# uci-cbcl/esm-efficient

Measured on AMD Instinct MI355X. Metric: residues/sec ESM2-650M fwd, 50k packed tokens; % bf16 MFMA peak; 1/2/4/8 GPU, higher is better.
Workload: dtype bf16

## Files before the change

### esm-efficient_amd/csrc/attn.hip

```cpp
#include "common.h"
#include "launch.h"
#include "gemm.h"

#include <atomic>
#include <type_traits>

namespace esme {

static constexpr int QT = 128;
static constexpr int KT = 64;
static constexpr int kAttnDma0 = 3, kAttnDma1 = 11;

struct AttnArgs {
    const u16* q; const u16* k; const u16* v; int64_t ld;
    u16* o; int64_t ldo;
    const int32_t* cu;
    int H;
    float scale_log2;
    int nqt;
    int nhb;
    float thr;
    int spec;
    const int32_t* order;
};

template <int D>
__device__ __forceinline__ int kswz(int row) {
    constexpr int CPR = D / 8;
    constexpr int RPB = 16 / CPR;
    return (row / RPB) & (CPR - 1);
}

template <int D, int QB, bool F16 = false>
__global__ __launch_bounds__(256, 2) void attn_varlen_kernel(const AttnArgs a) {
    constexpr int DS = D / 16;
    constexpr int DB = (D + 31) / 32;
    constexpr int CPR = D / 8;
    constexpr int KCH = KT * CPR;
    constexpr int KI = (KCH + 255) / 256;
    constexpr int DQ = D / 4;
    constexpr int DQ_HI_BITS = (D == 16 ? 0 : D == 32 ? 1 : D == 64 ? 2 : 3);
    constexpr int VI = (16 * DQ + 255) / 256;
    constexpr int K_BYTES = KT * D * 2;
    constexpr int BUF = K_BYTES + D * 128;
    const float THR = a.thr;

    __shared__ __attribute__((aligned(16))) char smem[2 * BUF];

    const int tid = threadIdx.x, lane = tid & 63, wave = tid >> 6;
    const int l31 = lane & 31, hi = lane >> 5;
    const int b = a.order ? a.order[blockIdx.z] : (int)blockIdx.z, h = blockIdx.y;
    const int s0 = a.cu[b], S = a.cu[b + 1] - s0;
    const int q0 = blockIdx.x * (QT * QB);
    if (q0 >= S) return;

    const unsigned int ld = (unsigned int)a.ld;
    const u16* qb = a.q + (int64_t)s0 * a.ld + h * D;
    const u16* kb = a.k + (int64_t)s0 * a.ld + h * D;
    const u16* vb = a.v + (int64_t)s0 * a.ld + h * D;

    int qrow[QB];
    bool blk_active[QB];
    bf16x8 qf[QB][DS];
#pragma unroll
    for (int b = 0; b < QB; ++b) {
        const int r0 = q0 + (wave * QB + b) * 32;
        qrow[b] = r0 + l31;
        blk_active[b] = r0 < S;
        const unsigned int qc = qrow[b] < S ? qrow[b] : S - 1;
#pragma unroll
        for (int ds = 0; ds < DS; ++ds)
            qf[b][ds] = *reinterpret_cast<const bf16x8*>(qb + (qc * ld + ds * 16 + hi * 8));
    }
    const bool wave_active = blk_active[0];

    unsigned int koff[KI];
    int krow[KI];
#pragma unroll
    for (int i = 0; i < KI; ++i) {
        const int c = i * 256 + tid;
        krow[i] = c / CPR;
        koff[i] = (unsigned int)(c % CPR) * 8u;
    }
    int v_dq[VI], v_kq[VI];
#pragma unroll
    for (int i = 0; i < VI; ++i) {
        const int rest = (lane >> 4) | (wave << 2) | (i << 4);
        v_dq[i] = (lane & 3) | ((rest & ((1 << DQ_HI_BITS) - 1)) << 2);
        v_kq[i] = ((lane >> 2) & 3) | ((rest >> DQ_HI_BITS) << 2);
    }
    u32x4 kreg[KI];
    u32x2 vreg[VI][4];
    auto load_tile = [&](int kv0) {
        const bool full = kv0 + KT <= S;
#pragma unroll
        for (int i = 0; i < KI; ++i) {
            if (KCH >= 256 * KI || krow[i] < KT) {
                unsigned int row = kv0 + krow[i];
                if (!full) row = row < (unsigned int)S ? row : S - 1;
                kreg[i] = *reinterpret_cast<const u32x4*>(kb + (row * ld + koff[i]));
            }
        }
#pragma unroll
        for (int i = 0; i < VI; ++i) {
            if (v_kq[i] < 16) {
#pragma unroll
                for (int kk = 0; kk < 4; ++kk) {
                    unsigned int row = kv0 + v_kq[i] * 4 + kk;
                    if (!full) row = row < (unsigned int)S ? row : S - 1;
                    vreg[i][kk] = *reinterpret_cast<const u32x2*>(vb + (row * ld + v_dq[i] * 4));
                }
            }
        }
    };
    auto store_tile = [&](char* Ks, char* Vt) {
#pragma unroll
        for (int i = 0; i < KI; ++i) {
            if (KCH >= 256 * KI || krow[i] < KT) {
                const int row = krow[i], ch = (int)(koff[i] >> 3);
                ESME_LDS_CHECK(Ks + row * (D * 2) + ((ch ^ kswz<D>(row)) << 4), 16, smem, 2 * BUF);
                *reinterpret_cast<u32x4*>(Ks + row * (D * 2) + ((ch ^ kswz<D>(row)) << 4)) = kreg[i];
            }
        }
#pragma unroll
        for (int i = 0; i < VI; ++i) {
            if (v_kq[i] < 16) {
                const int dq = v_dq[i], kq = v_kq[i];
#pragma unroll
                for (int dd = 0; dd < 4; ++dd) {
                    const int w = dd >> 1;
                    unsigned int e0, e1;
                    if (dd & 1) {
                        e0 = __builtin_amdgcn_perm(vreg[i][1][w], vreg[i][0][w], 0x07060302u);
                        e1 = __builtin_amdgcn_perm(vreg[i][3][w], vreg[i][2][w], 0x07060302u);
                    } else {
                        e0 = __builtin_amdgcn_perm(vreg[i][1][w], vreg[i][0][w], 0x05040100u);
                        e1 = __builtin_amdgcn_perm(vreg[i][3][w], vreg[i][2][w], 0x05040100u);
                    }
                    const int drow = dq * 4 + dd;
                    const int ch = kq >> 1;
                    u32x2 out = {e0, e1};
                    ESME_LDS_CHECK(Vt + drow * 128 + ((ch ^ ((drow >> 1) & 7)) << 4) + (kq & 1) * 8, 8, smem, 2 * BUF);
                    *reinterpret_cast<u32x2*>(Vt + drow * 128 + ((ch ^ ((drow >> 1) & 7)) << 4) + (kq & 1) * 8) = out;
                }
            }
        }
    };

    const int krow_perm = (l31 & 3) | (((l31 >> 3) & 1) << 2) | (((l31 >> 2) & 1) << 3) | (l31 & 16);

    f32x16 oacc[QB][DB];
    float mc[QB], l_run[QB];
#pragma unroll
    for (int b = 0; b < QB; ++b) {
        mc[b] = -1e30f; l_run[b] = 0.f;
#pragma unroll
        for (int i = 0; i < DB; ++i)
#pragma unroll
            for (int r = 0; r < 16; ++r) oacc[b][i][r] = 0.f;
    }
    const float c = a.scale_log2;

    const int ntiles = (S + KT - 1) / KT;
    load_tile(0);
// ... 242 lines not shown
                        const int drow = dq * 4 + dd;
                        const int ch = kq >> 1;
                        u32x2 out = {e0, e1};
                        ESME_LDS_CHECK(Vt + drow * 128 + ((ch ^ ((drow >> 1) & 7)) << 4) + (kq & 1) * 8, 8, smem, 2 * BUF);
                        *reinterpret_cast<u32x2*>(Vt + drow * 128 + ((ch ^ ((drow >> 1) & 7)) << 4) + (kq & 1) * 8) = out;
                    }
                }
            }
        }
    };

    const int krow_perm = (l31 & 3) | (((l31 >> 3) & 1) << 2) | (((l31 >> 2) & 1) << 3) | (l31 & 16);

    f32x16 oacc[DB];
    float mc = -1e30f, l_run = 0.f;
#pragma unroll
    for (int i = 0; i < DB; ++i)
#pragma unroll
        for (int r = 0; r < 16; ++r) oacc[i][r] = 0.f;
    const float c = a.scale_log2;

    const int ntiles = (S + KT - 1) / KT;
    load_tile(0);
    store_tile(smem);
    if (ntiles > 1) load_tile(KT);
    __syncthreads();
    for (int t = 0; t < ntiles; ++t) {
        const int kv0 = t * KT;
        const char* buf = smem + (t & 1) * BUF;
        if (wave_active) {
            f32x16 sacc[2];
#pragma unroll
            for (int kbk = 0; kbk < 2; ++kbk) {
#pragma unroll
                for (int r = 0; r < 16; ++r) sacc[kbk][r] = 0.f;
                const int row = kbk * 32 + krow_perm;
                const char* rp = buf + row * (D * 2);
                const int sw = kswz<D>(row);
#pragma unroll
                for (int ds = 0; ds < DS; ++ds) {
                    const bf16x8 kh = *reinterpret_cast<const bf16x8*>(rp + (((ds * 2 + hi) ^ sw) << 4));
                    ESME_LDS_CHECK(rp + K_BYTES + (((ds * 2 + hi) ^ sw) << 4), 16, smem, 2 * BUF);
                    const bf16x8 kl = *reinterpret_cast<const bf16x8*>(rp + K_BYTES + (((ds * 2 + hi) ^ sw) << 4));
                    sacc[kbk] = mfma_32x32x16<F16>(kl, qf[0][ds], sacc[kbk]);
                    sacc[kbk] = mfma_32x32x16<F16>(kh, qf[1][ds], sacc[kbk]);
                    sacc[kbk] = mfma_32x32x16<F16>(kh, qf[0][ds], sacc[kbk]);
                }
            }
            if (kv0 + KT > S) {
#pragma unroll
                for (int kbk = 0; kbk < 2; ++kbk)
#pragma unroll
                    for (int r = 0; r < 16; ++r)
                        if (kv0 + kbk * 32 + 16 * (r >> 3) + 8 * hi + (r & 7) >= S) sacc[kbk][r] = -1e30f;
            }
            float tmax = sacc[0][0];
#pragma unroll
            for (int r = 1; r < 16; ++r) tmax = fmaxf(tmax, sacc[0][r]);
#pragma unroll
            for (int r = 0; r < 16; ++r) tmax = fmaxf(tmax, sacc[1][r]);
            tmax = fmaxf(tmax, __shfl_xor(tmax, 32, 64));
            const float tmc = tmax * c;
            if (__any(tmc > mc)) {
                const float mn = fmaxf(mc, tmc);
                const float alpha = __builtin_amdgcn_exp2f(mc - mn);
                mc = mn;
                l_run *= alpha;
#pragma unroll
                for (int i = 0; i < DB; ++i)
#pragma unroll
                    for (int r = 0; r < 16; ++r) oacc[i][r] *= alpha;
            }
            bf16x8 pf[NPT][2][2];
            float psum = 0.f;
#pragma unroll
            for (int kbk = 0; kbk < 2; ++kbk)
#pragma unroll
                for (int s = 0; s < 2; ++s) {
                    float p[8], ph[8];
#pragma unroll
                    for (int j = 0; j < 8; ++j) {
                        p[j] = __builtin_amdgcn_exp2f(fmaf(sacc[kbk][8 * s + j], c, -mc));
                        psum += p[j];
                    }
                    const u32x4 pk = pack8t<F16>(p);
                    pf[0][kbk][s] = __builtin_bit_cast(bf16x8, pk);
                    if constexpr (!QKP) {
                        unpack8t<F16>(pk, ph);
#pragma unroll
                        for (int j = 0; j < 8; ++j) p[j] -= ph[j];
                        pf[NPT - 1][kbk][s] = __builtin_bit_cast(bf16x8, pack8t<F16>(p));
                    }
                }
            l_run += psum;

            const char* Vt = buf + 2 * K_BYTES;
#pragma unroll
            for (int i = 0; i < DB; ++i) {
                int drow = i * 32 + l31;
                if (D < 32) drow &= (D - 1);
                const char* rp = Vt + drow * 128;
                const int sw = (drow >> 1) & 7;
#pragma unroll
                for (int kbk = 0; kbk < 2; ++kbk)
#pragma unroll
                    for (int s = 0; s < 2; ++s) {
                        const bf16x8 vh = *reinterpret_cast<const bf16x8*>(rp + (((kbk * 4 + s * 2 + hi) ^ sw) << 4));
                        if constexpr (!QKP) {
                            ESME_LDS_CHECK(rp + V_BYTES + (((kbk * 4 + s * 2 + hi) ^ sw) << 4), 16, smem, 2 * BUF);
                            const bf16x8 vl = *reinterpret_cast<const bf16x8*>(rp + V_BYTES + (((kbk * 4 + s * 2 + hi) ^ sw) << 4));
                            oacc[i] = mfma_32x32x16<F16>(vl, pf[0][kbk][s], oacc[i]);
                            oacc[i] = mfma_32x32x16<F16>(vh, pf[NPT - 1][kbk][s], oacc[i]);
                        }
                        oacc[i] = mfma_32x32x16<F16>(vh, pf[0][kbk][s], oacc[i]);
                    }
            }
        }
        if (t + 1 < ntiles) {
            store_tile(smem + ((t + 1) & 1) * BUF);
            if (t + 2 < ntiles) load_tile(kv0 + 2 * KT);
        }
        __syncthreads();
    }

    if (!wave_active) return;
    const float l_tot = l_run + __shfl_xor(l_run, 32, 64);
    const float inv = 1.0f / l_tot;
    if (qrow < S) {
        u16* op = a.o + (int64_t)(s0 + qrow) * a.ldo + h * D;
#pragma unroll
        for (int i = 0; i < DB; ++i)
#pragma unroll
            for (int g = 0; g < 4; ++g) {
                const int d = i * 32 + 8 * g + 4 * hi;
                if (d < D) {
                    float o4[4];
#pragma unroll
                    for (int e = 0; e < 4; ++e) o4[e] = oacc[i][4 * g + e] * inv;
                    const u32x2 pk = {pack16<F16>(o4[0], o4[1]), pack16<F16>(o4[2], o4[3])};
                    *reinterpret_cast<u32x2*>(op + d) = pk;
                    if constexpr (!QKP) {
                        const u32x2 pl = {pack16<F16>(o4[0] - lo16<F16>(pk[0]), o4[1] - hi16<F16>(pk[0])), pack16<F16>(o4[2] - lo16<F16>(pk[1]), o4[3] - hi16<F16>(pk[1]))};
                        *reinterpret_cast<u32x2*>(op + sa.lo_out + d) = pl;
                    }
                }
            }
    }
}


template <int NW, bool QP = false, int D = 64, bool F16 = false>
__global__ __launch_bounds__(NW * 64, 2) void attn_pp64_kernel(const AttnArgs a) {
    constexpr float S0 = (QP && F16) ? -4.0f : 0.0f;
    constexpr int DS = D / 16, DB = D / 32, NT = NW * 64;
    constexpr int ROWB = D * 2;
    constexpr int K_BYTES = KT * D * 2;
    constexpr int SLOT = K_BYTES + D * 128;
    constexpr int ROWS = NW * 64;
    constexpr int NPV = 4 * DB, NQK = 2 * DS, NM = NPV + NQK;
    constexpr int PPS = 16 / NM;
    static_assert(D == 64 || D == 32, "head dims 64 and 32");
    static_assert(NW == 4 || (NW == 8 && D == 64), "4 waves (8: head dim 64 only)");
    extern __shared__ __attribute__((aligned(16))) char smem[];

    const int tid = threadIdx.x, lane = tid & 63;
    const int wave = __builtin_amdgcn_readfirstlane(tid >> 6);
    const int l31 = lane & 31, hi = lane >> 5;
    const unsigned int xcd = blockIdx.x & 7u, bi = blockIdx.x >> 3;
    const int qt = (int)(bi % (unsigned int)a.nqt);
    const unsigned int hb = (bi / (unsigned int)a.nqt) * 8u + xcd;
    if (hb >= (unsigned int)a.nhb) return;
    const int h = (int)(hb % (unsigned int)a.H), bi_seq = (int)(hb / (unsigned int)a.H);
    const int b = a.order ? a.order[bi_seq] : bi_seq;
    const int s0 = a.cu[b], S = a.cu[b + 1] - s0;
    const int q0 = qt * ROWS;
    if (q0 >= S) return;

    const unsigned int ld = (unsigned int)a.ld;
    const u16* qb = a.q + (int64_t)s0 * a.ld + h * D;
    const unsigned int kv_bytes = ((unsigned int)(S - 1) * ld + D) * 2u;
    auto make_rsrc = [&](const u16* p) -> u32x4 {
        const uint64_t v = (uint64_t)(uintptr_t)p;
        return u32x4{(unsigned int)__builtin_amdgcn_readfirstlane((int)(unsigned int)v),
                     (unsigned int)__builtin_amdgcn_readfirstlane((int)((unsigned int)(v >> 32) & 0xffffu)),
                     (unsigned int)__builtin_amdgcn_readfirstlane((int)kv_bytes), 0x00020000u};
    };
    const u32x4 krs = make_rsrc(a.k + (int64_t)s0 * a.ld + h * D);
    const u32x4 vrs = make_rsrc(a.v + (int64_t)s0 * a.ld + h * D);
    auto dma16 = [&](const u32x4 rs, const unsigned int voff, const char* dst) {
        ESME_LDS_CHECK(dst, 1024, smem, 4 * SLOT);
        const unsigned int d = (unsigned int)__builtin_amdgcn_readfirstlane((int)(unsigned int)(uintptr_t)dst);
        unsigned int keep;
        asm volatile("s_mov_b32 %0, m0\n\ts_mov_b32 m0, %2\n\ts_nop 0\n\tbuffer_load_dwordx4 %1, %3, 0 offen lds\n\ts_mov_b32 m0, %0"
                     : "=&s"(keep) : "v"(voff), "s"(d), "s"(rs) : "memory");
    };

    bf16x8 qf[2][DS];
    const int wrow0 = q0 + wave * 64;
    const bool wave_active = wrow0 < S;
#pragma unroll
    for (int bb = 0; bb < 2; ++bb) {
        const int qr = wrow0 + bb * 32 + l31;
        const unsigned int qc = qr < S ? qr : S - 1;
#pragma unroll
        for (int ds = 0; ds < DS; ++ds)
            qf[bb][ds] = *reinterpret_cast<const bf16x8*>(qb + (qc * ld + ds * 16 + hi * 8));
    }

    constexpr int KI = K_BYTES / (NW * 1024);
    constexpr int CPR = D / 8;
    const unsigned int tile_bytes = (unsigned int)KT * ld * 2u;
    unsigned int kg0, vg0;
    {
        const int r = wave * (64 / CPR) + lane / CPR, pch = lane % CPR;
        kg0 = ((unsigned int)r * ld + ((pch ^ kswz<D>(r)) * 8)) * 2u;
        vg0 = ((unsigned int)r * ld + ((D == 64 ? (pch ^ (((r >> 1) & 1) << 2)) : pch) * 8)) * 2u;
    }
    const unsigned int kg_step = (unsigned int)(NW * (64 / CPR)) * ld * 2u;
    auto dma_k = [&](int tile, char* slot) {
        const unsigned int base = (unsigned int)tile * tile_bytes + kg0;
#pragma unroll
        for (int i = 0; i < KI; ++i)
            dma16(krs, base + i * kg_step, slot + (i * NW + wave) * 1024);
    };
    auto dma_v = [&](int tile, char* slot) {
        const unsigned int base = (unsigned int)tile * tile_bytes + vg0;
#pragma unroll
        for (int i = 0; i < KI; ++i)
            dma16(vrs, base + i * kg_step, slot + K_BYTES + (i * NW + wave) * 1024);
    };

    const int krow_perm = (l31 & 3) | (((l31 >> 3) & 1) << 2) | (((l31 >> 2) & 1) << 3) | (l31 & 16);
    int kfo[DS];
#pragma unroll
    for (int i = 0; i < DS; ++i) kfo[i] = krow_perm * ROWB + (((i * 2 + hi) ^ kswz<D>(krow_perm)) << 4);
    int vb[DB];
    {
        const int j = (lane & 15) >> 2, p = lane & 3, gsel = (lane >> 4) & 1;
#pragma unroll
        for (int db = 0; db < DB; ++db) vb[db] = K_BYTES + (hi * 8 + j) * ROWB + (D == 64 ? ((db ^ (j >> 1)) * 64) : 0) + gsel * 32 + p * 8;
    }
    typedef short s16x4 __attribute__((ext_vector_type(4)));
    auto vfrag = [&](const char* Vs, const int db, const int ks) -> bf16x8 {
        typedef __attribute__((address_space(3))) s16x4* ltr_t;
        const char* p = Vs + vb[db] + ks * (16 * ROWB);
        ESME_LDS_CHECK(p, 8, smem, 4 * SLOT); ESME_LDS_CHECK(p + 4 * ROWB, 8, smem, 4 * SLOT);
        const s16x4 lo = __builtin_amdgcn_ds_read_tr16_b64_v4i16((ltr_t)(p));
        const s16x4 up = __builtin_amdgcn_ds_read_tr16_b64_v4i16((ltr_t)(p + 4 * ROWB));
        return __builtin_bit_cast(bf16x8, __builtin_shufflevector(lo, up, 0, 1, 2, 3, 4, 5, 6, 7));
    };

    f32x16 oacc[2][DB], sacc[2][2];
    u32x4 pw[2][2][2];
    float mc[2], lrun[2];
    const float c = a.scale_log2, thr = a.thr;
    int ovf = 0;

    auto frag = [&](int m, const char* Ks, const char* Vs) -> bf16x8 {
        if (m < NPV) return vfrag(Vs, m % DB, m / DB);
        ESME_LDS_CHECK(Ks + ((m - NPV) & 1) * (32 * ROWB) + kfo[(m - NPV) >> 1], 16, smem, 4 * SLOT);
        return *reinterpret_cast<const bf16x8*>(Ks + ((m - NPV) & 1) * (32 * ROWB) + kfo[(m - NPV) >> 1]);
    };

    f32x16 zneg = {S0, S0, S0, S0, S0, S0, S0, S0, S0, S0, S0, S0, S0, S0, S0, S0};
    if constexpr (QP && F16) asm volatile("" : "+v"(zneg));
    auto phase = [&](auto BS_, auto BM_, const bool need_max, const bool tail, const char* Ks, const char* Vs, const int kv0, auto&& hook) __attribute__((always_inline)) {
        constexpr int bs = decltype(BS_)::value, bm = decltype(BM_)::value;
        bf16x8 fr[3];
        fr[0] = frag(0, Ks, Vs);
        fr[1] = frag(1, Ks, Vs);
        auto mfma_step = [&](int m) {
            if (m + 2 < NM) fr[(m + 2) % 3] = frag(m + 2, Ks, Vs);
            if (m >= NPV) {
                const int j = m - NPV, kbk = j & 1, ds = j >> 1;
                if (ds == 0) {
                    if constexpr (QP && F16) {
                        sacc[bm][kbk] = mfma_32x32x16<F16>(fr[m % 3], qf[bm][ds], zneg);
                    } else {
                        const f32x16 z = {0.f, 0.f, 0.f, 0.f, 0.f, 0.f, 0.f, 0.f, 0.f, 0.f, 0.f, 0.f, 0.f, 0.f, 0.f, 0.f};
                        sacc[bm][kbk] = mfma_32x32x16<F16>(fr[m % 3], qf[bm][ds], z);
                    }
                } else {
                    sacc[bm][kbk] = mfma_32x32x16<F16>(fr[m % 3], qf[bm][ds], sacc[bm][kbk]);
                }
            } else {
                const int db = m % DB, ks = m / DB;
                oacc[bm][db] = mfma_32x32x16<F16>(
                    fr[m % 3], __builtin_bit_cast(bf16x8, pw[bm][ks >> 1][ks & 1]), oacc[bm][db]);
            }
        };
        float ps0, ps1, ps2, ps3;
        float xa0, xa1, pa0 = 0.f, pa1 = 0.f;
        auto pair_fma = [&](const int p, const float nm) {
            const int kbk = p >> 3, r = (2 * p) & 15;
            xa0 = fmaf(sacc[bs][kbk][r], c, nm);
            xa1 = fmaf(sacc[bs][kbk][r + 1], c, nm);
        };
        auto pair_sum_pack = [&](const int p, const float q0, const float q1) {
            const int kbk = p >> 3, r = (2 * p) & 15;
            pw[bs][kbk][r >> 3][(r & 7) >> 1] = pack16<F16>(q0, q1);
            if (p & 1) { ps2 += q0; ps3 += q1; } else { ps0 += q0; ps1 += q1; }
        };
        auto softmax_slot = [&](const int m, const float nm) {
            const float q0 = pa0, q1 = pa1;
            if constexpr (QP) {
                const int kb2 = m >> 3, r2 = (2 * m) & 15;
                pa0 = __builtin_amdgcn_exp2f(sacc[bs][kb2][r2]);
                pa1 = __builtin_amdgcn_exp2f(sacc[bs][kb2][r2 + 1]);
                if (m >= 1) pair_sum_pack(m - 1, q0, q1);
                const int pk = m >= 1 ? m - 1 : 0, kbk = pk >> 3, r = (2 * pk) & 15;
                asm volatile("" : "+v"(pw[bs][kbk][r >> 3]), "+v"(ps0), "+v"(ps1), "+v"(ps2), "+v"(ps3), "+v"(pa0), "+v"(pa1));
            } else {
                const float x0 = xa0, x1 = xa1;
                if (m + 1 < 16) pair_fma(m + 1, nm);
                pa0 = __builtin_amdgcn_exp2f(x0);
                pa1 = __builtin_amdgcn_exp2f(x1);
                if (m >= 1) pair_sum_pack(m - 1, q0, q1);
                const int pk = m >= 1 ? m - 1 : 0, kbk = pk >> 3, r = (2 * pk) & 15;
                asm volatile("" : "+v"(pw[bs][kbk][r >> 3]), "+v"(ps0), "+v"(ps1), "+v"(ps2), "+v"(ps3), "+v"(xa0), "+v"(xa1), "+v"(pa0), "+v"(pa1));
            }
        };
        auto tile_max = [&]() -> float {
            float tmax = sacc[bs][0][0];
#pragma unroll
            for (int r = 1; r < 16; ++r) tmax = fmaxf(tmax, sacc[bs][0][r]);
#pragma unroll
            for (int r = 0; r < 16; ++r) tmax = fmaxf(tmax, sacc[bs][1][r]);
            const auto sw = __builtin_amdgcn_permlane32_swap(__float_as_uint(tmax), __float_as_uint(tmax), false, false);
            return fmaxf(__uint_as_float(sw[0]), __uint_as_float(sw[1])) * c;
        };
        auto rescale_to = [&](const float tmc) {
            const float mn = fmaxf(mc[bs], tmc);
            const float alpha = __builtin_amdgcn_exp2f(mc[bs] - mn);
            mc[bs] = mn;
            lrun[bs] *= alpha;
#pragma unroll
            for (int i = 0; i < DB; ++i)
#pragma unroll
                for (int r = 0; r < 16; ++r) oacc[bs][i][r] *= alpha;
        };
        if (tail) {
            int lim = S - kv0 - 8 * hi;
            asm volatile("" : "+v"(lim));
#pragma unroll
            for (int kbk = 0; kbk < 2; ++kbk)
#pragma unroll
                for (int r = 0; r < 16; ++r)
                    if (kbk * 32 + 16 * (r >> 3) + (r & 7) >= lim) sacc[bs][kbk][r] = -1e30f;
        }
        if (need_max) {
            asm volatile("" ::: "memory");
            const float tmc = tile_max();
            if (__any(tmc > mc[bs] + thr)) rescale_to(tmc);
            if constexpr (QP) {
                const float mref = mc[bs];
#pragma unroll
                for (int kbk = 0; kbk < 2; ++kbk)
#pragma unroll
                    for (int r = 0; r < 16; ++r) sacc[bs][kbk][r] -= mref;
            }
        }
        ps0 = ps1 = ps2 = ps3 = 0.f;
        const float nm = -mc[bs];
        if constexpr (!QP) pair_fma(0, nm);
#pragma unroll
        for (int m = 0; m < NM; ++m) {
            mfma_step(m);
            __builtin_amdgcn_sched_barrier(0);
#pragma unroll
            for (int u = 0; u < PPS; ++u) softmax_slot(m * PPS + u, nm);
            hook(m);
            __builtin_amdgcn_sched_barrier(0);
        }
        pair_sum_pack(15, pa0, pa1);
        const float psum = (ps0 + ps1) + (ps2 + ps3);
        if (__any(!(psum < (F16 ? 3.0e4f : 1e30f)))) ovf = 1;
        lrun[bs] += psum;
    };
    using I0 = std::integral_constant<int, 0>;
    using I1 = std::integral_constant<int, 1>;

    const int nt = (S + KT - 1) / KT;
    bool exact = !a.spec;
    for (;;) {
    #pragma unroll
        for (int bb = 0; bb < 2; ++bb) {
            mc[bb] = -1e30f; lrun[bb] = (QP && !wave_active) ? 1e30f : 0.f;
    #pragma unroll
            for (int i = 0; i < 2; ++i) {
    #pragma unroll
                for (int r = 0; r < 16; ++r) { if (i < DB) oacc[bb][i < DB ? i : 0][r] = 0.f; sacc[bb][i][r] = S0; }
    #pragma unroll
                for (int s = 0; s < 2; ++s) pw[bb][i][s] = u32x4{0u, 0u, 0u, 0u};
            }
        }
        dma_k(0, smem);
        dma_v(0, smem);
        if (nt > 1) { dma_k(1, smem + SLOT); dma_v(1, smem + SLOT); }
        if (nt > 2) dma_k(2, smem + 2 * SLOT);
#pragma unroll
        for (int bb = 0; bb < 2; ++bb)
#pragma unroll
            for (int ds = 0; ds < DS; ds += 2) asm volatile("" : "+v"(qf[bb][ds]), "+v"(qf[bb][ds + 1]) : : "memory");
        {
            const u32x4 z = {0u, 0u, 0u, 0u};
            char* v3 = smem + 3 * SLOT + K_BYTES;
    #pragma unroll
            for (int i = 0; i < (D * 128) / (NT * 16); ++i) *reinterpret_cast<u32x4*>(v3 + (i * NT + tid) * 16) = z;
        }
        asm volatile("s_waitcnt vmcnt(0)" ::: "memory");
        __syncthreads();
        if (wave_active) {
    #pragma unroll
            for (int ds = 0; ds < DS; ++ds)
    #pragma unroll
                for (int kbk = 0; kbk < 2; ++kbk) {
                    const bf16x8 kf = *reinterpret_cast<const bf16x8*>(smem + kbk * (32 * ROWB) + kfo[ds]);
                    sacc[0][kbk] = mfma_32x32x16<F16>(kf, qf[0][ds], sacc[0][kbk]);
                }
        }
        const bool ragged = (S & (KT - 1)) != 0;
        auto dma_piece = [&](const unsigned int rs_sel, const int tile, char* slot, const int i) {
            if (rs_sel == 0) dma16(krs, (unsigned int)tile * tile_bytes + kg0 + i * kg_step, slot + (i * NW + wave) * 1024);
            else dma16(vrs, (unsigned int)tile * tile_bytes + vg0 + i * kg_step, slot + K_BYTES + (i * NW + wave) * 1024);
        };
        for (int t = 0; t < nt; ++t) {
            const bool pf_k = t + 3 < nt, pf_v = t + 2 < nt;
            char* kslot = smem + ((t + 3) & 3) * SLOT;
            char* vslot = smem + ((t + 2) & 3) * SLOT;
            if (wave_active) {
                const char* cur = smem + (t & 3) * SLOT;
                const char* prv = smem + ((t + 3) & 3) * SLOT;
                const char* nxt = smem + ((t + 1) & 3) * SLOT;
                const bool tail = t == nt - 1 && ragged;
                const bool need_max = exact || (!QP && t == 0);
                phase(I0{}, I1{}, need_max, tail, cur, prv, t * KT, [&](const int m) {
                    if (KI == 2) { if (m == kAttnDma0 && pf_k) dma_piece(0, t + 3, kslot, 0); if (m == kAttnDma1 && pf_k) dma_piece(0, t + 3, kslot, KI - 1); }
                    else if (m == NM / 2 - 1 && pf_k) dma_piece(0, t + 3, kslot, 0);
                });
                phase(I1{}, I0{}, need_max, tail, nxt, cur, t * KT, [&](const int m) {
                    if (KI == 2) { if (m == kAttnDma0 && pf_v) dma_piece(1, t + 2, vslot, 0); if (m == kAttnDma1 && pf_v) dma_piece(1, t + 2, vslot, KI - 1); }
                    else if (m == NM / 2 - 1 && pf_v) dma_piece(1, t + 2, vslot, 0);
                });
            } else {
                if (pf_k) dma_k(t + 3, kslot);
                if (pf_v) dma_v(t + 2, vslot);
            }
            if (t + 3 < nt) asm volatile("s_waitcnt vmcnt(%0) lgkmcnt(0)" :: "n"(2 * KI) : "memory");
            else if (t + 2 < nt) asm volatile("s_waitcnt vmcnt(%0) lgkmcnt(0)" :: "n"(KI) : "memory");
            else asm volatile("s_waitcnt vmcnt(0) lgkmcnt(0)" ::: "memory");
            __builtin_amdgcn_s_barrier();
        }
        if (wave_active) {
            const char* Vs = smem + ((nt - 1) & 3) * SLOT;
    #pragma unroll
            for (int ks = 0; ks < 4; ++ks)
    #pragma unroll
                for (int db = 0; db < DB; ++db) {
                    const bf16x8 vf = vfrag(Vs, db, ks);
                    oacc[1][db] = mfma_32x32x16<F16>(vf, __builtin_bit_cast(bf16x8, pw[1][ks >> 1][ks & 1]),
                                                                          oacc[1][db]);
                }
        }
        if constexpr (QP) {
            if (!exact) {
                const float vanish = F16 ? (float)S * 6.103515625e-5f : 1e-30f;
#pragma unroll
                for (int bb = 0; bb < 2; ++bb) {
                    const auto sw = __builtin_amdgcn_permlane32_swap(__float_as_uint(lrun[bb]), __float_as_uint(lrun[bb]), false, false);
                    if (__any(!(__uint_as_float(sw[0]) + __uint_as_float(sw[1]) > vanish))) ovf = 1;
                }
            }
        }
        if (exact || !__syncthreads_or(ovf)) break;
        exact = true;
        ovf = 0;
    }
    if (!wave_active) return;

    constexpr int OCH = D / 8;
    char* slab = smem + ((nt + (wave >> 2)) & 3) * SLOT + (wave & 3) * (32 * ROWB);
#pragma unroll
    for (int bb = 0; bb < 2; ++bb) {
        const auto sw = __builtin_amdgcn_permlane32_swap(__float_as_uint(lrun[bb]), __float_as_uint(lrun[bb]), false, false);
        const float inv = 1.0f / (__uint_as_float(sw[0]) + __uint_as_float(sw[1]));
        if (bb) __builtin_amdgcn_wave_barrier();
#pragma unroll
        for (int db = 0; db < DB; ++db)
#pragma unroll
            for (int g = 0; g < 4; ++g) {
                u32x2 pk = {pack16<F16>(oacc[bb][db][4 * g] * inv, oacc[bb][db][4 * g + 1] * inv),
                            pack16<F16>(oacc[bb][db][4 * g + 2] * inv, oacc[bb][db][4 * g + 3] * inv)};
                ESME_LDS_CHECK(slab + l31 * ROWB + (((db * 4 + g) ^ (l31 & (OCH - 1))) << 4) + hi * 8, 8, smem, 4 * SLOT);
                *reinterpret_cast<u32x2*>(slab + l31 * ROWB + (((db * 4 + g) ^ (l31 & (OCH - 1))) << 4) + hi * 8) = pk;
            }
        __builtin_amdgcn_wave_barrier();
        const int rbase = wrow0 + bb * 32;
#pragma unroll
        for (int it = 0; it < 32 / (64 / OCH); ++it) {
            const int r = it * (64 / OCH) + lane / OCH, ch = lane % OCH;
            ESME_LDS_CHECK(slab + r * ROWB + ((ch ^ (r & (OCH - 1))) << 4), 16, smem, 4 * SLOT);
            const u32x4 v = *reinterpret_cast<const u32x4*>(slab + r * ROWB + ((ch ^ (r & (OCH - 1))) << 4));
            if (rbase + r < S) *reinterpret_cast<u32x4*>(a.o + (int64_t)(s0 + rbase + r) * a.ldo + h * D + ch * 8) = v;
        }
    }
}


template <int D, bool F16, bool QKP, bool QP>
__global__ __launch_bounds__(256, 2) void attn_sb_kernel(const AttnSplitArgs sa) {
    static_assert(!QKP || F16, "q/k pairs: the fp16 form");
    static_assert(!(F16 && QP), "fp16 P needs a reference maximum");
    static_assert(D == 64 || D == 32, "head dims 64 and 32");
    const AttnArgs& a = sa.a;
    constexpr int NW = 4, NT = 256, DS = D / 16, DB = D / 32;
    constexpr int ROWB = D * 2, K_BYTES = KT * D * 2, KP = QKP ? 2 : 1;
    constexpr int V_OFF = KP * K_BYTES, SLOT = V_OFF + D * 128, NS = 3, ROWS = NW * 32;
    constexpr int NPV = 4 * DB, NQK1 = 2 * DS, NQK = NQK1 * (QKP ? 3 : 1), NM = NPV + NQK;
    extern __shared__ __attribute__((aligned(16))) char smem_sb[];
    char* smem = smem_sb;

    const int tid = threadIdx.x, lane = tid & 63;
    const int wave = __builtin_amdgcn_readfirstlane(tid >> 6);
    const int l31 = lane & 31, hi = lane >> 5;
    const unsigned int xcd = blockIdx.x & 7u, bi = blockIdx.x >> 3;
    const int qt = (int)(bi % (unsigned int)a.nqt);
    const unsigned int hb = (bi / (unsigned int)a.nqt) * 8u + xcd;
    if (hb >= (unsigned int)a.nhb) return;
    const int h = (int)(hb % (unsigned int)a.H), bi_seq = (int)(hb / (unsigned int)a.H);
    const int b = a.order ? a.order[bi_seq] : bi_seq;
    const int s0 = a.cu[b], S = a.cu[b + 1] - s0;
    const int q0 = qt * ROWS;
    if (q0 >= S) return;

    const unsigned int ld = (unsigned int)a.ld;
    const u16* qb = a.q + (int64_t)s0 * a.ld + h * D;
    const unsigned int kv_bytes = ((unsigned int)(S - 1) * ld + D) * 2u;
    auto make_rsrc = [&](const u16* p) -> u32x4 {
        const uint64_t v = (uint64_t)(uintptr_t)p;
        return u32x4{(unsigned int)__builtin_amdgcn_readfirstlane((int)(unsigned int)v),
                     (unsigned int)__builtin_amdgcn_readfirstlane((int)((unsigned int)(v >> 32) & 0xffffu)),
                     (unsigned int)__builtin_amdgcn_readfirstlane((int)kv_bytes), 0x00020000u};
    };
    const u32x4 krs = make_rsrc(a.k + (int64_t)s0 * a.ld + h * D);
    const u32x4 klrs = make_rsrc(a.k + (QKP ? sa.lo_in : 0) + (int64_t)s0 * a.ld + h * D);
    const u32x4 vrs = make_rsrc(a.v + (int64_t)s0 * a.ld + h * D);
    auto dma16 = [&](const u32x4 rs, const unsigned int voff, const char* dst) {
        ESME_LDS_CHECK(dst, 1024, smem, NS * SLOT);
        const unsigned int d = (unsigned int)__builtin_amdgcn_readfirstlane((int)(unsigned int)(uintptr_t)dst);
        unsigned int keep;
        asm volatile("s_mov_b32 %0, m0\n\ts_mov_b32 m0, %2\n\ts_nop 0\n\tbuffer_load_dwordx4 %1, %3, 0 offen lds\n\ts_mov_b32 m0, %0"
                     : "=&s"(keep) : "v"(voff), "s"(d), "s"(rs) : "memory");
    };

    bf16x8 qf[DS], qfl[QKP ? DS : 1];
    const int wrow0 = q0 + wave * 32;
    const bool wave_active = wrow0 < S;
    {
        const int qr = wrow0 + l31;
        const unsigned int qc = qr < S ? qr : S - 1;
#pragma unroll
        for (int ds = 0; ds < DS; ++ds) {
            qf[ds] = *reinterpret_cast<const bf16x8*>(qb + (qc * ld + ds * 16 + hi * 8));
            if constexpr (QKP) qfl[ds] = *reinterpret_cast<const bf16x8*>(qb + sa.lo_in + (qc * ld + ds * 16 + hi * 8));
        }
    }

    constexpr int KI = K_BYTES / (NW * 1024);
    constexpr int CPR = D / 8;
    const unsigned int tile_bytes = (unsigned int)KT * ld * 2u;
    unsigned int kg0, vg0;
    {
        const int r = wave * (64 / CPR) + lane / CPR, pch = lane % CPR;
        kg0 = ((unsigned int)r * ld + ((pch ^ kswz<D>(r)) * 8)) * 2u;
        vg0 = ((unsigned int)r * ld + ((D == 64 ? (pch ^ (((r >> 1) & 1) << 2)) : pch) * 8)) * 2u;
    }
    const unsigned int kg_step = (unsigned int)(NW * (64 / CPR)) * ld * 2u;
    auto dma_k_piece = [&](const int tile, char* slot, const int p) {
        const int part = p / KI, i = p % KI;
        dma16(part ? klrs : krs, (unsigned int)tile * tile_bytes + kg0 + i * kg_step, slot + part * K_BYTES + (i * NW + wave) * 1024);
    };
    auto dma_v_piece = [&](const int tile, char* slot, const int i) {
        dma16(vrs, (unsigned int)tile * tile_bytes + vg0 + i * kg_step, slot + V_OFF + (i * NW + wave) * 1024);
    };
    auto dma_k = [&](const int tile, char* slot) {
#pragma unroll
        for (int p = 0; p < KP * KI; ++p) dma_k_piece(tile, slot, p);
    };
    auto dma_v = [&](const int tile, char* slot) {
#pragma unroll
        for (int i = 0; i < KI; ++i) dma_v_piece(tile, slot, i);
    };

    const int krow_perm = (l31 & 3) | (((l31 >> 3) & 1) << 2) | (((l31 >> 2) & 1) << 3) | (l31 & 16);
    int kfo[DS];
#pragma unroll
    for (int i = 0; i < DS; ++i) kfo[i] = krow_perm * ROWB + (((i * 2 + hi) ^ kswz<D>(krow_perm)) << 4);
    int vb[DB];
    {
        const int j = (lane & 15) >> 2, p = lane & 3, gsel = (lane >> 4) & 1;
#pragma unroll
        for (int db = 0; db < DB; ++db) vb[db] = V_OFF + (hi * 8 + j) * ROWB + (D == 64 ? ((db ^ (j >> 1)) * 64) : 0) + gsel * 32 + p * 8;
    }
    typedef short s16x4 __attribute__((ext_vector_type(4)));
    auto vfrag = [&](const char* Vs, const int db, const int ks) -> bf16x8 {
        typedef __attribute__((address_space(3))) s16x4* ltr_t;
        const char* p = Vs + vb[db] + ks * (16 * ROWB);
        ESME_LDS_CHECK(p, 8, smem, NS * SLOT); ESME_LDS_CHECK(p + 4 * ROWB, 8, smem, NS * SLOT);
        const s16x4 lo = __builtin_amdgcn_ds_read_tr16_b64_v4i16((ltr_t)(p));
        const s16x4 up = __builtin_amdgcn_ds_read_tr16_b64_v4i16((ltr_t)(p + 4 * ROWB));
        return __builtin_bit_cast(bf16x8, __builtin_shufflevector(lo, up, 0, 1, 2, 3, 4, 5, 6, 7));
    };

    f32x16 oacc[DB], sacc[2][2];
    u32x4 pw[2][2][2];
    float mc, lrun;
    const float c = a.scale_log2, thr = a.thr;
    int ovf = 0;

    auto frag = [&](const int m, const char* Ks, const char* Vs) -> bf16x8 {
        if (m < NPV) return vfrag(Vs, m % DB, m / DB);
        const int j = (m - NPV) % NQK1, pass = (m - NPV) / NQK1;
        const char* p = Ks + (pass == 1 ? K_BYTES : 0) + (j & 1) * (32 * ROWB) + kfo[j >> 1];
        ESME_LDS_CHECK(p, 16, smem, NS * SLOT);
        return *reinterpret_cast<const bf16x8*>(p);
    };

    auto phase = [&](auto P_, const bool need_max, const bool tail, const char* Ks, const char* Vs, const int kv0, auto&& hook) __attribute__((always_inline)) {
        constexpr int P = decltype(P_)::value, PN = P ^ 1;
        bf16x8 fr[3];
        fr[0] = frag(0, Ks, Vs);
        fr[1] = frag(1, Ks, Vs);
        auto mfma_step = [&](const int m) {
            if (m + 2 < NM) fr[(m + 2) % 3] = frag(m + 2, Ks, Vs);
            if (m >= NPV) {
                const int j = (m - NPV) % NQK1, pass = (m - NPV) / NQK1, kbk = j & 1, ds = j >> 1;
                const bf16x8 qop = (QKP && pass == 2) ? qfl[QKP ? ds : 0] : qf[ds];
                if (pass == 0 && ds == 0) {
                    const f32x16 z = {0.f, 0.f, 0.f, 0.f, 0.f, 0.f, 0.f, 0.f, 0.f, 0.f, 0.f, 0.f, 0.f, 0.f, 0.f, 0.f};
                    sacc[PN][kbk] = mfma_32x32x16<F16>(fr[m % 3], qop, z);
                } else {
                    sacc[PN][kbk] = mfma_32x32x16<F16>(fr[m % 3], qop, sacc[PN][kbk]);
                }
            } else {
                const int db = m % DB, ks = m / DB;
                oacc[db] = mfma_32x32x16<F16>(fr[m % 3], __builtin_bit_cast(bf16x8, pw[PN][ks >> 1][ks & 1]), oacc[db]);
            }
        };
        float ps0, ps1, ps2, ps3;
        float xa0, xa1, pa0 = 0.f, pa1 = 0.f;
        auto pair_fma = [&](const int p, const float nm) {
            const int kbk = p >> 3, r = (2 * p) & 15;
            xa0 = fmaf(sacc[P][kbk][r], c, nm);
            xa1 = fmaf(sacc[P][kbk][r + 1], c, nm);
        };
        auto pair_sum_pack = [&](const int p, const float q0_, const float q1_) {
            const int kbk = p >> 3, r = (2 * p) & 15;
            pw[P][kbk][r >> 3][(r & 7) >> 1] = pack16<F16>(q0_, q1_);
            if (p & 1) { ps2 += q0_; ps3 += q1_; } else { ps0 += q0_; ps1 += q1_; }
// ... 406 lines not shown
```

Measured before the change: 807,900.

## Carry softmax tail and next V fragments across attention phases

```diff
diff --git a/esm-efficient_amd/csrc/attn.hip b/esm-efficient_amd/csrc/attn.hip
--- a/esm-efficient_amd/csrc/attn.hip
+++ b/esm-efficient_amd/csrc/attn.hip
@@ -10,6 +10,16 @@
 static constexpr int QT = 128;
 static constexpr int KT = 64;
 static constexpr int kAttnDma0 = 3, kAttnDma1 = 11;
+
+#ifdef ESME_ATTN_TRACE
+static constexpr bool kAttnTrace = true;
+static constexpr int kAttnTraceBlocks = 4096, kAttnTraceWords = 24;
+__device__ unsigned long long g_attn_trace[kAttnTraceBlocks * 4 * kAttnTraceWords];
+#else
+static constexpr bool kAttnTrace = false;
+#endif
+#define ESME_ATTN_SEG(i) do { if constexpr (kAttnTrace) { unsigned long long now_; ESME_ATTN_STAMP(now_); tr_acc[i] += (unsigned int)now_ - tr_last; tr_last = (unsigned int)now_; } } while (0)
+#define ESME_ATTN_STAMP(x) do { if constexpr (kAttnTrace) { __builtin_amdgcn_sched_barrier(0); asm volatile("s_memtime %0\n\ts_waitcnt lgkmcnt(0)" : "=s"(x) :: "memory"); __builtin_amdgcn_sched_barrier(0); } } while (0)
 
 struct AttnArgs {
     const u16* q; const u16* k; const u16* v; int64_t ld;
@@ -558,6 +568,11 @@
 template <int NW, bool QP = false, int D = 64, bool F16 = false>
 __global__ __launch_bounds__(NW * 64, 2) void attn_pp64_kernel(const AttnArgs a) {
     constexpr float S0 = (QP && F16) ? -4.0f : 0.0f;
+#ifdef ESME_ATTN_OLD_PHASE_ORDER
+    constexpr bool kReorder = false;
+#else
+    constexpr bool kReorder = !(QP && F16 && D == 64);
+#endif
     constexpr int DS = D / 16, DB = D / 32, NT = NW * 64;
     constexpr int ROWB = D * 2;
     constexpr int K_BYTES = KT * D * 2;
@@ -572,6 +587,9 @@
     const int tid = threadIdx.x, lane = tid & 63;
     const int wave = __builtin_amdgcn_readfirstlane(tid >> 6);
     const int l31 = lane & 31, hi = lane >> 5;
+    [[maybe_unused]] unsigned long long tr_entry = 0, tr_cal = 0, tr_loop0 = 0, tr_loop1 = 0, tr_exit = 0;
+    [[maybe_unused]] unsigned int tr_acc[9] = {0u, 0u, 0u, 0u, 0u, 0u, 0u, 0u, 0u}, tr_last = 0u;
+    ESME_ATTN_STAMP(tr_entry);
     const unsigned int xcd = blockIdx.x & 7u, bi = blockIdx.x >> 3;
     const int qt = (int)(bi % (unsigned int)a.nqt);
     const unsigned int hb = (bi / (unsigned int)a.nqt) * 8u + xcd;
@@ -670,13 +688,25 @@
 
     f32x16 zneg = {S0, S0, S0, S0, S0, S0, S0, S0, S0, S0, S0, S0, S0, S0, S0, S0};
     if constexpr (QP && F16) asm volatile("" : "+v"(zneg));
-    auto phase = [&](auto BS_, auto BM_, const bool need_max, const bool tail, const char* Ks, const char* Vs, const int kv0, auto&& hook) __attribute__((always_inline)) {
+    bf16x8 hf0 = {}, hf1 = {};
+    float tps0 = 0.f, tps1 = 0.f, tps2 = 0.f, tps3 = 0.f, tpa0 = 0.f, tpa1 = 0.f;
+    auto carry_finish = [&](auto B_) {
+        constexpr int bq = decltype(B_)::value;
+        pw[bq][1][1][3] = pack16<F16>(tpa0, tpa1);
+        tps2 += tpa0; tps3 += tpa1;
+        const float psum = (tps0 + tps1) + (tps2 + tps3);
+        if (__any(!(psum < (F16 ? 3.0e4f : 1e30f)))) ovf = 1;
+        lrun[bq] += psum;
+    };
+    auto phase = [&](auto BS_, auto BM_, const bool need_max, const bool tail, const char* Ks, const char* Vs, const char* nVs, const int kv0, const int seg0, auto&& hook) __attribute__((always_inline)) {
         constexpr int bs = decltype(BS_)::value, bm = decltype(BM_)::value;
+        ESME_ATTN_SEG(seg0);
         bf16x8 fr[3];
-        fr[0] = frag(0, Ks, Vs);
-        fr[1] = frag(1, Ks, Vs);
+        if constexpr (kReorder) { fr[0] = hf0; fr[1] = hf1; }
+        else { fr[0] = frag(0, Ks, Vs); fr[1] = frag(1, Ks, Vs); }
         auto mfma_step = [&](int m) {
             if (m + 2 < NM) fr[(m + 2) % 3] = frag(m + 2, Ks, Vs);
+            else if constexpr (kReorder) { if (m + 2 == NM) hf0 = frag(0, Ks, nVs); else hf1 = frag(1, Ks, nVs); }
             if (m >= NPV) {
                 const int j = m - NPV, kbk = j & 1, ds = j >> 1;
                 if (ds == 0) {
@@ -769,19 +799,20 @@
         ps0 = ps1 = ps2 = ps3 = 0.f;
         const float nm = -mc[bs];
         if constexpr (!QP) pair_fma(0, nm);
+        ESME_ATTN_SEG(seg0 + 1);
 #pragma unroll
         for (int m = 0; m < NM; ++m) {
             mfma_step(m);
+            if (m == 0) ESME_ATTN_SEG(seg0 + 2);
             __builtin_amdgcn_sched_barrier(0);
 #pragma unroll
             for (int u = 0; u < PPS; ++u) softmax_slot(m * PPS + u, nm);
+            if constexpr (kReorder) { if (m == 1) carry_finish(BM_); }
             hook(m);
             __builtin_amdgcn_sched_barrier(0);
         }
-        pair_sum_pack(15, pa0, pa1);
-        const float psum = (ps0 + ps1) + (ps2 + ps3);
-        if (__any(!(psum < (F16 ? 3.0e4f : 1e30f)))) ovf = 1;
-        lrun[bs] += psum;
+        tps0 = ps0; tps1 = ps1; tps2 = ps2; tps3 = ps3; tpa0 = pa0; tpa1 = pa1;
+        if constexpr (!kReorder) carry_finish(BS_);
     };
     using I0 = std::integral_constant<int, 0>;
     using I1 = std::integral_constant<int, 1>;
@@ -816,7 +847,9 @@
         }
         asm volatile("s_waitcnt vmcnt(0)" ::: "memory");
         __syncthreads();
+        tps0 = tps1 = tps2 = tps3 = tpa0 = tpa1 = 0.f;
         if (wave_active) {
+            if constexpr (kReorder) { hf0 = frag(0, smem, smem + 3 * SLOT); hf1 = frag(1, smem, smem + 3 * SLOT); }
     #pragma unroll
             for (int ds = 0; ds < DS; ++ds)
     #pragma unroll
@@ -826,44 +859,62 @@
                 }
         }
         const bool ragged = (S & (KT - 1)) != 0;
+        ESME_ATTN_STAMP(tr_loop0);
+        tr_last = (unsigned int)tr_loop0;
         auto dma_piece = [&](const unsigned int rs_sel, const int tile, char* slot, const int i) {
             if (rs_sel == 0) dma16(krs, (unsigned int)tile * tile_bytes + kg0 + i * kg_step, slot + (i * NW + wave) * 1024);
             else dma16(vrs, (unsigned int)tile * tile_bytes + vg0 + i * kg_step, slot + K_BYTES + (i * NW + wave) * 1024);
         };
+        auto tile_end = [&](const int t) __attribute__((always_inline)) {
+            constexpr int LG = kReorder ? 4 : 0;
+            if (t + 3 < nt) asm volatile("s_waitcnt vmcnt(%0) lgkmcnt(%1)" :: "n"(2 * KI), "n"(LG) : "memory");
+            else if (t + 2 < nt) asm volatile("s_waitcnt vmcnt(%0) lgkmcnt(%1)" :: "n"(KI), "n"(LG) : "memory");
+            else asm volatile("s_waitcnt vmcnt(0) lgkmcnt(%0)" :: "n"(LG) : "memory");
+            __builtin_amdgcn_s_barrier();
+        };
+        if (kReorder && !wave_active) {
+            for (int t = 0; t < nt; ++t) {
+                if (t + 3 < nt) dma_k(t + 3, smem + ((t + 3) & 3) * SLOT);
+                if (t + 2 < nt) dma_v(t + 2, smem + ((t + 2) & 3) * SLOT);
+                tile_end(t);
+            }
+        } else
         for (int t = 0; t < nt; ++t) {
             const bool pf_k = t + 3 < nt, pf_v = t + 2 < nt;
             char* kslot = smem + ((t + 3) & 3) * SLOT;
             char* vslot = smem + ((t + 2) & 3) * SLOT;
-            if (wave_active) {
+            if (kReorder || wave_active) {
                 const char* cur = smem + (t & 3) * SLOT;
                 const char* prv = smem + ((t + 3) & 3) * SLOT;
                 const char* nxt = smem + ((t + 1) & 3) * SLOT;
                 const bool tail = t == nt - 1 && ragged;
                 const bool need_max = exact || (!QP && t == 0);
-                phase(I0{}, I1{}, need_max, tail, cur, prv, t * KT, [&](const int m) {
+                phase(I0{}, I1{}, need_max, tail, cur, prv, cur, t * KT, 0, [&](const int m) {
                     if (KI == 2) { if (m == kAttnDma0 && pf_k) dma_piece(0, t + 3, kslot, 0); if (m == kAttnDma1 && pf_k) dma_piece(0, t + 3, kslot, KI - 1); }
                     else if (m == NM / 2 - 1 && pf_k) dma_piece(0, t + 3, kslot, 0);
                 });
-                phase(I1{}, I0{}, need_max, tail, nxt, cur, t * KT, [&](const int m) {
+                ESME_ATTN_SEG(3);
+                phase(I1{}, I0{}, need_max, tail, nxt, cur, cur, t * KT, 4, [&](const int m) {
                     if (KI == 2) { if (m == kAttnDma0 && pf_v) dma_piece(1, t + 2, vslot, 0); if (m == kAttnDma1 && pf_v) dma_piece(1, t + 2, vslot, KI - 1); }
                     else if (m == NM / 2 - 1 && pf_v) dma_piece(1, t + 2, vslot, 0);
                 });
+                ESME_ATTN_SEG(7);
             } else {
                 if (pf_k) dma_k(t + 3, kslot);
                 if (pf_v) dma_v(t + 2, vslot);
             }
-            if (t + 3 < nt) asm volatile("s_waitcnt vmcnt(%0) lgkmcnt(0)" :: "n"(2 * KI) : "memory");
-            else if (t + 2 < nt) asm volatile("s_waitcnt vmcnt(%0) lgkmcnt(0)" :: "n"(KI) : "memory");
-            else asm volatile("s_waitcnt vmcnt(0) lgkmcnt(0)" ::: "memory");
-            __builtin_amdgcn_s_barrier();
-        }
+            tile_end(t);
+            if (wave_active) ESME_ATTN_SEG(8);
+        }
+        ESME_ATTN_STAMP(tr_loop1);
         if (wave_active) {
             const char* Vs = smem + ((nt - 1) & 3) * SLOT;
+            if constexpr (kReorder) carry_finish(I1{});
     #pragma unroll
             for (int ks = 0; ks < 4; ++ks)
     #pragma unroll
                 for (int db = 0; db < DB; ++db) {
-                    const bf16x8 vf = vfrag(Vs, db, ks);
+                    const bf16x8 vf = (kReorder && ks * DB + db < 2) ? (ks * DB + db == 0 ? hf0 : hf1) : vfrag(Vs, db, ks);
                     oacc[1][db] = mfma_32x32x16<F16>(vf, __builtin_bit_cast(bf16x8, pw[1][ks >> 1][ks & 1]),
                                                                           oacc[1][db]);
                 }
@@ -910,7 +961,33 @@
             if (rbase + r < S) *reinterpret_cast<u32x4*>(a.o + (int64_t)(s0 + rbase + r) * a.ldo + h * D + ch * 8) = v;
         }
     }
-}
+#ifdef ESME_ATTN_TRACE
+    if constexpr (NW == 4) {
+        unsigned int hwid, xcc;
+        asm volatile("s_getreg_b32 %0, hwreg(HW_REG_HW_ID)\n\ts_getreg_b32 %1, hwreg(20)" : "=s"(hwid), "=s"(xcc));
+        asm volatile("s_waitcnt vmcnt(0)" ::: "memory");
+        ESME_ATTN_STAMP(tr_cal);
+        ESME_ATTN_STAMP(tr_exit);
+        if (lane == 0 && blockIdx.x < (unsigned int)kAttnTraceBlocks) {
+            unsigned long long* w = g_attn_trace + ((size_t)blockIdx.x * 4 + wave) * kAttnTraceWords;
+            w[0] = tr_entry; w[1] = tr_loop0; w[2] = tr_loop1; w[3] = tr_exit;
+            w[9] = tr_exit - tr_cal; w[10] = (unsigned long long)nt; w[11] = hwid; w[12] = xcc; w[13] = (unsigned long long)S; w[14] = exact ? 1u : 0u; w[15] = 1u;
+            for (int i = 0; i < 9; ++i) w[i < 5 ? 4 + i : 11 + i] = tr_acc[i];
+        }
+    }
+#endif
+}
+
+#ifdef ESME_ATTN_TRACE
+extern "C" int esme_hip_debug_read_attn_trace(void* dst, size_t bytes) {
+    if (bytes > sizeof(g_attn_trace)) return -1;
+    if (hipDeviceSynchronize() != hipSuccess) return -2;
+    if (hipMemcpyFromSymbol(dst, HIP_SYMBOL(g_attn_trace), bytes) != hipSuccess) return -3;
+    void* p = nullptr;
+    if (hipGetSymbolAddress(&p, HIP_SYMBOL(g_attn_trace)) != hipSuccess || hipMemset(p, 0, sizeof(g_attn_trace)) != hipSuccess) return -4;
+    return 0;
+}
+#endif
 
 
 template <int D, bool F16, bool QKP, bool QP>
```

Measured after the change: 808,400 (median of 3 runs). No clear change (+0.1%).
